# lightbulb128/troy

Hardware: AMD Instinct MI355X
Metric: ct x ct multiply+relinearize ops/sec, BFV N=2^15 L=14; achieved HBM GB/s vs peak (higher is better)
Workload: dtype u64; 1 GPU; bfv_n32768_l14; scheme=BFV, N=32768, K=15, L=14, batch_per_gpu=256, parallelism=batch-shard x1, streams_per_gpu=2, Bsk=15, limb_transforms_per_op=443

## Files before the change

### troy_amd/csrc/bfly.h

```cpp
#pragma once
#include "modarith.h"

namespace troyhip {

struct PrimeConst { u64 p, two_p, three_p, four_p, negp; };
__device__ __forceinline__ PrimeConst make_prime_const(u64 p) { return PrimeConst{p, 2 * p, 3 * p, 4 * p, 0 - p}; }

__device__ __forceinline__ u32 lo32(u64 x) { return (u32)x; }
__device__ __forceinline__ u32 hi32(u64 x) { return (u32)(x >> 32); }
__device__ __forceinline__ u64 mk64(u32 lo, u32 hi) { return ((u64)hi << 32) | lo; }

#ifdef TROYHIP_CPU_EMUL
__device__ __forceinline__ void csub4(u64 (&x)[4], u64 m) { for (int i = 0; i < 4; i++) x[i] = x[i] >= m ? x[i] - m : x[i]; }
__device__ __forceinline__ void sub4(u64 (&r)[4], const u64 (&a)[4], const u64 (&b)[4]) { for (int i = 0; i < 4; i++) r[i] = a[i] - b[i]; }
__device__ __forceinline__ u64 mulhi_approx1(u64 y, u64 wq) {
    const u64 y0 = lo32(y), y1 = hi32(y), q0 = lo32(wq), q1 = hi32(wq);
    const u128 s = (u128)(y1 * q0) + (u128)(y0 * q1);
    return y1 * q1 + (u64)(s >> 32);
}
__device__ __forceinline__ void mulhi_approx4(u64 (&q)[4], const u64 (&y)[4], const Shoup (&w)[4]) { for (int i = 0; i < 4; i++) q[i] = mulhi_approx1(y[i], w[i].quo); }
__device__ __forceinline__ u64 mul_acc(u64 acc, u64 y, u64 w, u64 q, u64 negp) { return acc + w * y + q * negp; }
__device__ __forceinline__ void mulhi_approx4_u(u64 (&q)[4], const u64 (&y)[4], const Shoup (&w)[4]) { mulhi_approx4(q, y, w); }
__device__ __forceinline__ u64 mul_acc_u(u64 acc, u64 y, u64 w, u64 q, u64 negp) { return mul_acc(acc, y, w, q, negp); }
__device__ __forceinline__ u64 mul_acc0(u64 y, u64 w, u64 q, u64 negp) { return mul_acc(0, y, w, q, negp); }
// ... 254 lines not shown
#pragma unroll
    for (int i = 0; i < 4; i++) {
        const u32 q = (u32)(((u64)hi32(x[i]) * mu) >> 32);
        x[i] += (u64)q * c.negp;
    }
}
__device__ __forceinline__ void lite_reduce1(u64 &x, u32 mu, const PrimeConst &c) {
    const u32 q = (u32)(((u64)hi32(x) * mu) >> 32);
    x += (u64)q * c.negp;
}
struct LeanFinal { unsigned sh; u32 mu; };
__device__ __forceinline__ LeanFinal make_lean_final(u64 p, u64 cr1) {
    const int b = 64 - __builtin_clzll(p);
    return LeanFinal{(unsigned)(b - 26), (u32)(cr1 >> (58 - b))};
}
__device__ __forceinline__ void lean_final4(u64 (&x)[4], const LeanFinal f, const PrimeConst &c) {
#pragma unroll
    for (int i = 0; i < 4; i++) {
        const u32 q = (u32)(((u64)(u32)(x[i] >> f.sh) * f.mu) >> 32);
        x[i] += (u64)q * c.negp;
    }
    csub4(x, c.p);
}
template <int NV> __device__ __forceinline__ void lean_final(u64 (&x)[NV], const LeanFinal f, const PrimeConst &c) {
#pragma unroll
    for (int h = 0; h < NV / 4; h++) {
        u64 v[4] = {x[4 * h], x[4 * h + 1], x[4 * h + 2], x[4 * h + 3]};
        lean_final4(v, f, c);
#pragma unroll
        for (int i = 0; i < 4; i++) x[4 * h + i] = v[i];
    }
}
__device__ __forceinline__ void reduce4_from_8p(u64 (&x)[4], const PrimeConst &c) { csub4(x, c.four_p); csub4(x, c.two_p); csub4(x, c.p); }
__device__ __forceinline__ void reduce4_from_4p(u64 (&x)[4], const PrimeConst &c) { csub4(x, c.two_p); csub4(x, c.p); }


struct Acc128 { u32 a0, a1, a2, a3; };
// ... 81 lines not shown
```

### troy_amd/csrc/evaluator.cpp

```cpp
#include "evaluator.h"
#include "hostcrypto.h"
#include "kernels.h"
#include <algorithm>
#include <cmath>
#include <cstdlib>
#include <cstring>

namespace troyhip {

static bool tensor_fused() {
    static const bool v = [] { const char *e = probe_env("TROYHIP_TENSOR"); return !(e && e[0] == 's'); }();
    return v;
}
static bool ks_fused() {
    static const bool v = [] { const char *e = probe_env("TROYHIP_KS"); return !(e && e[0] == 's'); }();
    return v;
}

static bool ks_moddown_fused() {
    static const bool v = [] { const char *e = probe_env("TROYHIP_MODDOWN"); return !(e && e[0] == 's'); }();
    return v;
}

static bool corr_fused() {
// ... 141 lines not shown
    u64 new_cf = a.cf;
    const bool same = (a.data == b.data && a.bstride == b.bstride && sa == sb);
    auto dense = [&](u64 bstride, u64 words) { return batch == 1 || bstride == words; };

    if (c.scheme == SCHEME_BFV) {
        if (a.ntt || b.ntt) throw Error(ST_INVALID_ARGUMENT, "encrypted1 or encrypted2 cannot be in NTT form");
        const Level &lv = c.level(L);
        const int nb = (int)lv.rns.Bsk.size();
        const u64 bw = (u64)nb * N;
        const int sp = sa + sb;
        u64 *xq = c.arena.take(batch * sp * pw), *xb = c.arena.take(batch * sp * bw);
        u64 *dq = c.arena.take(batch * ds * pw), *db = c.arena.take(batch * ds * bw);
        const LimbMap bmap = c.ids_map(lv.bsk_ids);
        const bool merged = dense(a.bstride, (u64)sa * pw) && dense(b.bstride, (u64)sb * pw) && sa == 2 && sb == 2 && ntt2_tensor_supported(c.logn) && tensor_fused() &&
                            L + nb <= 64 && take_merged(c, batch * sp * (u64)(L + nb));
        bool all_done = false;
        if (merged) {
            const u64 mw = (u64)(L + nb) * N;
            std::vector<uint8_t> ids;
            for (int l = 0; l < L; l++) ids.push_back((uint8_t)l);
            ids.insert(ids.end(), lv.bsk_ids.begin(), lv.bsk_ids.end());
            const LimbMap mmap = c.ids_map(ids);
            u64 *X = xq, *D = dq;
            if (xb != xq + batch * sp * pw || db != dq + batch * ds * pw) throw Error(ST_LOGIC_ERROR, "multiply: the merged scratch is not contiguous (arena alignment changed?)");
            u64 *X_b = same ? X : X + batch * sa * mw;
            if (same || batch * sp > 65535) {
                launch_behz_extend(a.data, pw, X + (u64)L * N, mw, c.d_desc, *lv.behz, N, batch * sa, s);
                if (!same) launch_behz_extend(b.data, pw, X_b + (u64)L * N, mw, c.d_desc, *lv.behz, N, batch * sb, s);
            } else launch_behz_extend(a.data, pw, X + (u64)L * N, mw, c.d_desc, *lv.behz, N, batch * sp, s, b.data, batch * sa);
            launch_ntt2_tensor(X, a.data, X_b, b.data, D, c.d_desc, mmap, batch, c.logn, s, (unsigned)L);
            const PrimeDesc *idesc = behz_floor_prescaled(*lv.behz) ? lv.behz->floor_desc : c.d_desc;
            launch_ntt(D, idesc, mmap, batch * ds * (u64)(L + nb), c.logn, true, s);
            u64 *res = dense(out.bstride, (u64)ds * pw) ? out.data : X;
            launch_behz_floor_sk(D, mw, D + (u64)L * N, mw, res, pw, c.d_desc, *lv.behz, N, batch * ds, s);
            if (res != out.data) launch_copy_strided(res, ds * pw, out.data, out.bstride, ds * pw, batch, s);
            all_done = true;
        } else if (dense(a.bstride, (u64)sa * pw) && dense(b.bstride, (u64)sb * pw)) {
            const bool fused = sa == 2 && sb == 2 && ntt2_tensor_supported(c.logn) && tensor_fused();
            const bool once = same && fused;
            u64 *xq_a = xq, *xq_b = once ? xq : xq + batch * sa * pw, *xb_a = xb, *xb_b = once ? xb : xb + batch * sa * bw;
            launch_behz_extend(a.data, pw, xb_a, bw, c.d_desc, *lv.behz, N, batch * sa, s);
            if (!once) launch_behz_extend(b.data, pw, xb_b, bw, c.d_desc, *lv.behz, N, batch * sb, s);
            if (fused) {
                launch_ntt2_tensor(xq_a, a.data, xq_b, b.data, dq, c.d_desc, qmap, batch, c.logn, s);
                launch_ntt2_tensor(xb_a, nullptr, xb_b, nullptr, db, c.d_desc, bmap, batch, c.logn, s);
            } else {
                launch_ntt_from(xq_a, a.data, c.d_desc, qmap, batch * sa * L, c.logn, s);
                launch_ntt_from(xq_b, b.data, c.d_desc, qmap, batch * sb * L, c.logn, s);
                launch_ntt(xb, c.d_desc, bmap, batch * sp * nb, c.logn, false, s);
                launch_tensor(sa, sb, xq_a, xq_b, dq, sa * pw, sb * pw, c.d_desc, qmap, c.logn, L, batch, s);
                launch_tensor(sa, sb, xb_a, xb_b, db, sa * bw, sb * bw, c.d_desc, bmap, c.logn, nb, batch, s);
            }
        } else {
            launch_copy_strided(a.data, a.bstride, xq, sp * pw, sa * pw, batch, s);
            launch_copy_strided(b.data, b.bstride, xq + sa * pw, sp * pw, sb * pw, batch, s);
            launch_behz_extend(xq, pw, xb, bw, c.d_desc, *lv.behz, N, batch * sp, s);
            launch_ntt(xq, c.d_desc, qmap, batch * sp * L, c.logn, false, s);
            launch_ntt(xb, c.d_desc, bmap, batch * sp * nb, c.logn, false, s);
            launch_tensor(sa, sb, xq, xq + sa * pw, dq, sp * pw, sp * pw, c.d_desc, qmap, c.logn, L, batch, s);
            launch_tensor(sa, sb, xb, xb + sa * bw, db, sp * bw, sp * bw, c.d_desc, bmap, c.logn, nb, batch, s);
        }
        if (!all_done) {
            const PrimeDesc *idesc = behz_floor_prescaled(*lv.behz) ? lv.behz->floor_desc : c.d_desc;
            launch_ntt(dq, idesc, qmap, batch * ds * L, c.logn, true, s);
            launch_ntt(db, idesc, bmap, batch * ds * nb, c.logn, true, s);
        }
        if (all_done) {
        } else if (dense(out.bstride, (u64)ds * pw)) {
            launch_behz_floor_sk(dq, pw, db, bw, out.data, pw, c.d_desc, *lv.behz, N, batch * ds, s);
        } else {
            u64 *res = xq;
            launch_behz_floor_sk(dq, pw, db, bw, res, pw, c.d_desc, *lv.behz, N, batch * ds, s);
            launch_copy_strided(res, ds * pw, out.data, out.bstride, ds * pw, batch, s);
        }
    } else if (c.scheme == SCHEME_CKKS) {
        if (!(a.ntt && b.ntt)) throw Error(ST_INVALID_ARGUMENT, "encrypted1 or encrypted2 must be in NTT form");
        new_scale = a.scale * b.scale;
        if (!scale_ok(new_scale, L)) throw Error(ST_INVALID_ARGUMENT, "scale out of bounds");
        if (out.data != a.data && out.data != b.data && dense(out.bstride, (u64)ds * pw)) {
            launch_tensor(sa, sb, a.data, b.data, out.data, a.bstride, b.bstride, c.d_desc, qmap, c.logn, L, batch, s);
// ... 673 lines not shown
```

### troy_amd/csrc/kernels.h

```cpp
#pragma once
#include "device_types.h"

namespace troyhip {

unsigned device_cus();
inline unsigned plan_per_workgroup(size_t units, unsigned cap, size_t groups) {
    const size_t want = 4 * (size_t)device_cus();
    unsigned r = cap ? cap : 1;
    while (r > 1 && ((units + r - 1) / r) * groups < want) r = (r + 1) / 2;
    return r;
}

void launch_ntt(u64 *data, const PrimeDesc *primes, const LimbMap &map, size_t rows, int logn, bool inverse, hipStream_t stream);
bool ntt2_tensor_supported(int logn);
bool ntt2_ks_mac_supported(int logn);
void launch_ntt2_tensor(u64 *xa, const u64 *src_a, u64 *xb, const u64 *src_b, u64 *out, const PrimeDesc *primes, const LimbMap &map, size_t batch, int logn,
                        hipStream_t stream, unsigned src_slots = 0);
void launch_ntt_from(u64 *data, const u64 *src, const PrimeDesc *primes, const LimbMap &map, size_t rows, int logn, hipStream_t stream);

struct KsBase { const u64 *ptr = nullptr; u64 bstride = 0; int polys = 1; };

bool ntt2_supported(int logn);
struct Ntt2ModDown { int kind; u64 *ct; u64 ct_bstride; unsigned dl; u64 qk, half; const u64 *share; KsBase base; };
enum class Ntt2Source {
    SAME_LAYOUT,
    KS_DIGITS
};
enum class Ntt2Passes { BOTH, FIRST, SECOND };
enum : unsigned { NTT_ALL_SLOTS = ~0u };
struct Ntt2Request {
    u64 *data;
    const PrimeDesc *primes;
    LimbMap map;
    size_t rows;
    int logn;
    bool inverse = false;
    struct {
        const u64 *ptr = nullptr;
        Ntt2Source kind = Ntt2Source::SAME_LAYOUT;
        u64 ostride = 0;
        u64 bound = 0;
    } src;
    unsigned slot_begin = 0, slot_count = NTT_ALL_SLOTS;
    Ntt2Passes passes = Ntt2Passes::BOTH;
    unsigned plan_begin = 0, plan_count = 0;
    const Ntt2ModDown *md = nullptr;
};
void launch_ntt2(const Ntt2Request &r, hipStream_t stream);
struct KsArgs;
void launch_ntt2_ks_mac(u64 *D, const u64 *src, u64 src_ostride, const LimbMap &map, size_t rows, const u64 *key, u64 *acc, const u64 *ckks_target, u64 t_bstride,
                        bool lazy, u64 src_bound, const KsArgs &a, hipStream_t stream);

enum class Ntt1Feature { PLAIN , MOD_DOWN , CORRECTION , STRIDED_INVERSE };
bool ntt1_supported(int logn, const LimbMap &map, size_t rows, Ntt1Feature feature = Ntt1Feature::PLAIN);
struct Ntt1ModDown { u64 *ct; u64 ct_bstride; u64 dl, qk, half; KsBase base; };
struct Ntt1Corr {
    const u64 *last, *in;
    u64 in_ostride;
    u64 *out;
    u64 out_gstride, out_ostride;
    unsigned group;
// ... 3 lines not shown
    u64 in_gstride = 0;
    KsBase base;
};
struct Ntt1Request {
    const PrimeDesc *primes;
    LimbMap map;
    size_t rows;
    int logn;
    u64 *data = nullptr;
    bool inverse = false;
    const u64 *src = nullptr;
    u64 src_ostride = 0;
    u64 slot_mask = ~0ull;
    const Ntt1ModDown *md = nullptr;
    const Ntt1Corr *cr = nullptr;
};
void launch_ntt1(const Ntt1Request &r, hipStream_t stream);

void launch_ew(int op, const u64 *a, const u64 *b, u64 *out, const PrimeDesc *primes, const LimbMap &map, int logn, u64 rows, hipStream_t s);
void launch_mul_scalar(u64 *x, const PrimeDesc *primes, const LimbMap &map, const u64 *scalars, int logn, u64 rows, hipStream_t s);
void launch_mul_plain(u64 *a, const u64 *plain, const PrimeDesc *primes, const LimbMap &map, int logn, u64 limbs, u64 rows, hipStream_t s,
                      u64 rows_per_item = 0, u64 plain_bstride = 0);

struct PlainArgs {
    const PrimeDesc *primes;
    LimbMap map;
    u64 delta[64];
    u64 t_p, t_cr0, t_cr1;
    u64 q_mod_t, thr;
    u64 cf;
// ... 211 lines not shown
```

### troy_amd/csrc/ntt.hip

```cpp
#include "kernels.h"

namespace troyhip {

struct NttArgs {
    u64 *data;
    const PrimeDesc *primes;
    LimbMap map;
    int logn;
    int logT;
    int s_first;
    int n_stages;
    int logC;
    int lps;
    int strided;
    int tiles_per_row_log;
    int final_pass;
};

#define NTT_THREADS 256

__device__ __forceinline__ u64 gidx(const NttArgs &a, unsigned tile, unsigned f) {
    unsigned base = a.strided ? (tile << a.logC) : (tile << a.logT);
    return ((u64)(f >> a.logC) << a.lps) + base + (f & ((1u << a.logC) - 1));
}
// ... 126 lines not shown
            }
            v.x = v.x >= p ? v.x - p : v.x;
            v.y = v.y >= p ? v.y - p : v.y;
        }
        *reinterpret_cast<ulonglong2 *>(x + gidx(a, tile, f)) = v;
    }
}

static void plan(int logn, int &k1, int &k2) {
    if (logn <= 11) { k1 = 0; k2 = logn; return; }
    k2 = 9;
    if (logn - k2 > 7) k2 = logn - 7;
    k1 = logn - k2;
}

static bool launch_production(u64 *data, const u64 *src, const PrimeDesc *primes, const LimbMap &map, size_t rows, int logn, bool inverse, hipStream_t stream) {
    if (ntt1_supported(logn, map, rows)) {
        Ntt1Request q{primes, map, rows, logn};
        q.data = data;
        q.src = src;
        q.inverse = inverse;
        launch_ntt1(q, stream);
        return true;
    }
    if (!ntt2_supported(logn) || rows % ((size_t)map.period * map.inner)) return false;
    Ntt2Request q{data, primes, map, rows, logn};
    q.src.ptr = src;
    q.inverse = inverse;
    launch_ntt2(q, stream);
    return true;
}
void launch_ntt_from(u64 *data, const u64 *src, const PrimeDesc *primes, const LimbMap &map, size_t rows, int logn, hipStream_t stream) {
    if (rows == 0 || launch_production(data, src, primes, map, rows, logn, false, stream)) return;
    HIP_CHECK(hipMemcpyAsync(data, src, (rows << logn) * sizeof(u64), hipMemcpyDeviceToDevice, stream));
    launch_ntt(data, primes, map, rows, logn, false, stream);
}
void launch_ntt(u64 *data, const PrimeDesc *primes, const LimbMap &map, size_t rows, int logn, bool inverse, hipStream_t stream) {
    if (rows == 0 || launch_production(data, nullptr, primes, map, rows, logn, inverse, stream)) return;
    int k1, k2;
    plan(logn, k1, k2);
    NttArgs a;
    a.data = data;
    a.primes = primes;
    a.map = map;
    a.logn = logn;
    a.logT = logn < 11 ? logn : 11;
    a.tiles_per_row_log = logn - a.logT;
    unsigned blocks = (unsigned)(rows << a.tiles_per_row_log);
    auto strided = [&](bool final_pass) {
        a.strided = 1; a.n_stages = k1; a.logC = a.logT - k1; a.lps = logn - k1; a.final_pass = final_pass;
        a.s_first = inverse ? k1 - 1 : 0;
    };
    auto contiguous = [&](bool final_pass) {
// ... 18 lines not shown
```

### troy_amd/csrc/ntt1.hip

```cpp
#include "kernels.h"
#include <atomic>
#include "bfly.h"
#include "fpmod.h"
#include <cstdio>
#include <cstdlib>
#include <cstring>
#include <type_traits>

namespace troyhip {

#define N1_THREADS 1024
#define N1_LOGN 15
#define N1_N (1u << N1_LOGN)

struct Ntt1Args {
    u64 *data;
    const u64 *src;
    u64 src_ostride;
    const PrimeDesc *primes;
    LimbMap map;
    unsigned m_total;
    unsigned rows_per_wg;
    unsigned chunks;
    unsigned nslots;
// ... 1033 lines not shown
        else return ntt1s_fwd_kernel<LOGN, LEAN>;
    }
}
void launch_ntt1(const Ntt1Request &r, hipStream_t stream) {
    const LimbMap &map = r.map;
    const int logn = r.logn;
    const bool inverse = r.inverse;
    const Ntt1ModDown *md = r.md;
    const Ntt1Corr *cr = r.cr;
    if (r.rows == 0) return;
    if (logn < 12 || logn > N1_LOGN) throw Error(ST_LOGIC_ERROR, "ntt1: unsupported size");
    if (logn != N1_LOGN && (cr || (r.src && inverse))) throw Error(ST_LOGIC_ERROR, "ntt1: the correction form and the strided source belong to N = 2^15");
    const size_t per_outer = (size_t)map.period * map.inner;
    if (r.rows % per_outer) throw Error(ST_INVALID_ARGUMENT, "ntt1: row count must be a multiple of the limb pattern");
    if (md && (!inverse || map.inner != 1 || md->dl >= map.period)) throw Error(ST_LOGIC_ERROR, "ntt1: the mod-down epilogue belongs to the inverse transform of [..][slot][N] accumulators");
    Ntt1Args a;
    std::memset(&a, 0, sizeof(a));
    a.data = r.data;
    a.src = r.src;
    a.src_ostride = r.src_ostride;
    if (r.src && inverse && !r.src_ostride) throw Error(ST_LOGIC_ERROR, "ntt1: the out-of-place inverse takes a strided source");
    a.primes = r.primes;
    a.map = map;
    a.m_total = (unsigned)(r.rows / per_outer * map.inner);
    if (cr) {
        if (inverse || map.inner != 1 || r.src) throw Error(ST_LOGIC_ERROR, "ntt1: the correction form belongs to the forward transform of [outer][slot][N] rows");
        a.cr_last = cr->last; a.cr_in = cr->in; a.cr_out = cr->out; a.cr_inv = cr->inv;
        a.cr_in_ostride = cr->in_ostride; a.cr_in_gstride = cr->in_gstride; a.cr_out_gstride = cr->out_gstride; a.cr_out_ostride = cr->out_ostride;
        a.cr_qx = cr->qx; a.cr_half = cr->half; a.cr_group = cr->group ? cr->group : 1; a.cr_accumulate = cr->accumulate ? 1 : 0;
        a.cr_base = cr->base.ptr; a.cr_base_gstride = cr->base.bstride; a.cr_base_polys = cr->base.polys;
// ... 88 lines not shown
```

### troy_amd/csrc/ntt2.hip

```cpp
#include "kernels.h"
#include "bfly.h"
#include "fpmod.h"
#include <cstdio>
#include <cstdlib>
#include <cstring>
#include <type_traits>

namespace troyhip {

#define N2_THREADS 256
#define N2_LOGT 11
#define N2_T 2048

struct Ntt2Args {
    u64 *data;
    const u64 *src;
    u64 src_ostride;
    const PrimeDesc *primes;
    LimbMap map;
    int logn;
    unsigned tiles_per_row_log;
    unsigned m_total;
    unsigned rows_per_wg;
    unsigned chunks;
    int src_reduce;
    u64 src_bound;
    int slot_fastest;
    int src_same_layout;
    const u64 *src2;
    unsigned src_slots, src_split;
    u64 *tensor_b;
    u64 *tensor_out;
    const u64 *mac_key;
    u64 *mac_acc;
    const u64 *mac_target;
    u64 mac_tstride;
    unsigned mac_K;
    int mac_lazy;
    uint8_t mac_key_limb[65];
    unsigned slot_begin = 0;
    u64 *md_ct = nullptr;
    u64 md_ct_bstride = 0, md_qk = 0, md_half = 0;
    const u64 *md_share = nullptr;
    const u64 *md_base = nullptr;
    u64 md_base_bstride = 0;
    int md_base_polys = 1;
    int skip_diag = 0;
// ... 208 lines not shown
    __device__ static __forceinline__ void stage_read(u64 (&x)[8], const u64 *wave_stage) {
        const unsigned lane = threadIdx.x & 63;
        if (INV) {
            const u64 *mine = wave_stage + 128 * (lane >> 4) + 2 * (lane & 15);
#pragma unroll
            for (int j = 0; j < 4; j++) {
                const ulonglong2 v = *reinterpret_cast<const ulonglong2 *>(mine + 32 * j);
                x[2 * j] = v.x;
                x[2 * j + 1] = v.y;
            }
        } else {
#pragma unroll
            for (int e = 0; e < 8; e++) x[e] = wave_stage[lane + 64 * e];
        }
    }
    __device__ static __forceinline__ void store_via_lds(const u64 (&x)[8], u64 *row, unsigned tile, u64 *wave_xchg) {
        const unsigned lane = threadIdx.x & 63, w = threadIdx.x >> 6;
        u64 *mine = wave_xchg + 128 * (lane >> 4) + 2 * (lane & 15);
#pragma unroll
        for (int j = 0; j < 4; j++) {
            ulonglong2 v;
            v.x = x[2 * j];
            v.y = x[2 * j + 1];
            *reinterpret_cast<ulonglong2 *>(mine + 32 * j) = v;
        }
        TROY_WAVE_SYNC();
        u64 *dst = row + ((size_t)tile << N2_LOGT) + 512 * w + 2 * unit_perm(lane);
#pragma unroll
        for (int c = 0; c < 4; c++) {
            const ulonglong2 v = *reinterpret_cast<const ulonglong2 *>(wave_xchg + 128 * c + 2 * lane);
            *reinterpret_cast<ulonglong2 *>(dst + 128 * c) = v;
        }
    }
    __device__ static __forceinline__ void tensor_epilogue(u64 (&x)[8], u64 (&tx)[3][8], unsigned mm, u64 *out, unsigned period, unsigned slot, unsigned tile, int logn,
                                                           const Mod &m, u64 *xchg, const bool lean, const FpPrime *fc = nullptr) {
        const PrimeConst pc = make_prime_const(m.p);
        if (fc) {
#pragma unroll
            for (int e = 0; e < 8; e++) x[e] = fp_canonical(fp_of_bits(x[e]), *fc, m.p);
        } else if (lean) {
#pragma unroll
            for (int h = 0; h < 2; h++) {
                u64 v[4] = {x[4 * h], x[4 * h + 1], x[4 * h + 2], x[4 * h + 3]};
                lite_reduce4(v, (u32)m.cr1, pc);
#pragma unroll
                for (int i = 0; i < 4; i++) x[4 * h + i] = v[i];
            }
        } else {
#pragma unroll
            for (int h = 0; h < 2; h++) {
                u64 v[4] = {x[4 * h], x[4 * h + 1], x[4 * h + 2], x[4 * h + 3]};
                reduce4_from_8p(v, pc);
#pragma unroll
                for (int i = 0; i < 4; i++) x[4 * h + i] = v[i];
            }
        }
        const unsigned vr = mm & 3;
        if (vr < 3) {
#pragma unroll
            for (int i = 0; i < 3; i++)
                if ((int)vr == i) {
#pragma unroll
                    for (int e = 0; e < 8; e++) tx[i][e] = x[e];
                }
            return;
        }
        const unsigned b = mm >> 2;
        const ProdMod pm = make_prod_mod(m);
        u64 d[3][8];
#pragma unroll
        for (int e = 0; e < 8; e++) {
            const u64 a0 = tx[0][e], a1 = tx[1][e], b0 = tx[2][e], b1 = x[e];
            d[0][e] = reduce_prod((u128)a0 * b0, pm);
            d[1][e] = reduce_prod((u128)a0 * b1 + (u128)a1 * b0, pm);
            d[2][e] = reduce_prod((u128)a1 * b1, pm);
        }
#pragma unroll
        for (int i = 0; i < 3; i++) {
            u64 *orow = out + ((((u64)b * 3 + i) * period + slot) << logn);
            if (xchg) {
                TROY_WAVE_SYNC();
                store_via_lds(d[i], orow, tile, xchg + 512 * (threadIdx.x >> 6));
                continue;
            }
            ulonglong2 *op = reinterpret_cast<ulonglong2 *>(orow + ((u64)tile << N2_LOGT) + 8 * threadIdx.x);
#pragma unroll
            for (int e = 0; e < 4; e++) {
                ulonglong2 v;
                v.x = d[i][2 * e];
                v.y = d[i][2 * e + 1];
                op[e] = v;
            }
        }
    }
    template <int REDUCE> __device__ static __forceinline__ void g_read(u64 (&x)[8], const u64 *row, unsigned tile, int logn, const Mod &m, const unsigned t = threadIdx.x) {
#pragma unroll
        for (int u = 0; u < G; u++) {
            const unsigned q = t + THREADS * u;
            if (LOGD == 0) {
#pragma unroll
                for (int e = 0; e < (1 << R); e += 2) {
                    const ulonglong2 v = *reinterpret_cast<const ulonglong2 *>(row + g_index<STRIDED, NS, LOGC>(tile, elem(q, e), logn));
                    x[(u << R) + e] = v.x;
                    x[(u << R) + e + 1] = v.y;
                }
// ... 180 lines not shown
        }
        const u64 r = ((u64)o * period + slot) * inner + k;
        row = a.data + (r << logn);
        in = (REDUCE || a.src) ? (a.src_same_layout ? a.src + (r << logn) : a.src + (u64)o * a.src_ostride + ((u64)k << logn)) : row;
        if constexpr (!REDUCE && STRIDED && !INV) {
            if (a.src_same_layout == 2)
                in = slot >= a.src_slots ? row : (o < a.src_split ? a.src + (((u64)o * a.src_slots + slot) << logn) : a.src2 + (((u64)(o - a.src_split) * a.src_slots + slot) << logn));
        }
    };
    constexpr bool DMA = WAVE_PRIVATE;
    static_assert(MAC != 3 || DMA, "the CKKS key-switch pass (MAC = 3) takes its rows from the LDS-DMA staging area");
    constexpr bool PF = STRIDED && !INV && NR == 2 && !REDUCE;
    u64 xn[PF ? 8 : 1];
    static_assert(!MAC || (!INV && !STRIDED && NS == 9), "the inner product is fused into the forward contiguous pass");
    u64 tx[MAC == 2 ? 3 : 1][8];
    Acc128 macc[2][2][4];
    double facc[2][FP ? 8 : 1];
    auto mac_row = [&](const u64 (&xr)[8], const ulonglong2 (&kw)[2][KS ? 4 : 1], unsigned row_no) {
        if constexpr (FP && KS) {
#pragma unroll
            for (int cpt = 0; cpt < 2; cpt++)
#pragma unroll
                for (int e = 0; e < 8; e++) {
                    const u64 kword = (e & 1) ? kw[cpt][e >> 1].y : kw[cpt][e >> 1].x;
                    facc[cpt][e] += fp_mulmod_pinv(fp_of_bits(xr[e]), fp_from_u64(kword), fc);
                }
            if (a.fp_acc_every && (row_no + 1) % a.fp_acc_every == 0) {
#pragma unroll
                for (int cpt = 0; cpt < 2; cpt++)
#pragma unroll
// ... 2 lines not shown
        } else if constexpr (KS) {
#pragma unroll
            for (int cpt = 0; cpt < 2; cpt++) {
#pragma unroll
                for (int g = 0; g < 2; g++) {
                    const ulonglong2 k01 = kw[cpt][2 * g], k23 = kw[cpt][2 * g + 1];
                    const u64 kk[4] = {k01.x, k01.y, k23.x, k23.y};
                    const u64 xx[4] = {xr[4 * g], xr[4 * g + 1], xr[4 * g + 2], xr[4 * g + 3]};
                    mac128x4(macc[cpt][g], xx, kk);
                }
            }
        }
        (void)row_no;
    };
    constexpr bool MAC_STORE_LINEAR = KS && WAVE_PRIVATE;
    u64 *const wave_stage = lds[1] + 512 * (threadIdx.x >> 6);
    constexpr bool KSU = MAC != 0 && !FP;
    const unsigned units = KSU ? (a.mac_units ? a.mac_units : 1u) : 1u;
    const unsigned groups = KSU && a.mac_groups ? a.mac_groups : a.chunks * units;
    const unsigned last_group = chunk * units + units < groups ? chunk * units + units : groups;
    const unsigned stage_end = KSU ? last_group * a.rows_per_wg : 0;
    for (unsigned un = 0; un < units; un++) {
        const unsigned uchunk = KSU ? chunk * units + un : chunk;
        if (KSU && uchunk >= groups) break;
        const unsigned m_begin = uchunk * a.rows_per_wg;
        const unsigned m_end = (m_begin + a.rows_per_wg < a.m_total) ? m_begin + a.rows_per_wg : a.m_total;
        if (KS) {
#pragma unroll
            for (int cpt = 0; cpt < 2; cpt++)
#pragma unroll
                for (int g = 0; g < 2; g++)
// ... 132 lines not shown
                        Rd0::template g_read<REDUCE>(xn, nin, tile, logn, m, n2_opaque(threadIdx.x));
                    }
                }
                fp_guard(x, 1);
                if constexpr (FP) Rd1::compute_fp(x, tw1, fc, pd.inv_n); else Rd1::compute(x, tw1, pd, lean);
                if constexpr (NR == 2) {
                    if constexpr (FINAL >= 3) Rd1::template md_write<FINAL>(x, a, mm, slot, tile, logn, m, pd, fcp);
                    else Rd1::template g_write<FINAL>(x, row, tile, logn, m, lean, nullptr, fcp);
                } else {
                    Rd1::lds_write(x, buf, (FRESH & 4) ? n2_opaque(threadIdx.x) : threadIdx.x);
                    round_sync();
                    Rd2::lds_read(x, buf, (FRESH & 8) ? n2_opaque(threadIdx.x) : threadIdx.x);
                    fp_guard(x, 2);
                    if constexpr (FP) Rd2::compute_fp(x, tw2, fc, pd.inv_n); else Rd2::compute(x, tw2, pd, lean);
                    if constexpr (NR == 3 && MAC == 2) {
                        Rd2::tensor_epilogue(x, tx, mm, a.tensor_out, period, slot, tile, logn, m, WAVE_PRIVATE ? buf : nullptr, lean, fcp);
                    } else if constexpr (NR == 3 && KS) {
                        if constexpr (FP) {
                        } else if (!a.mac_lazy && lean) {
#pragma unroll
                            for (int e = 0; e < 8; e++) x[e] = barrett64(x[e], m);
                        } else if (!a.mac_lazy) {
                            const PrimeConst pc = make_prime_const(pd.p);
#pragma unroll
                            for (int h = 0; h < 2; h++) {
                                u64 v[4] = {x[4 * h], x[4 * h + 1], x[4 * h + 2], x[4 * h + 3]};
                                reduce4_from_8p(v, pc);
#pragma unroll
                                for (int i = 0; i < 4; i++) x[4 * h + i] = v[i];
                            }
                        }
// ... 28 lines not shown
            if (!skip_row) parity ^= 1u;
        }
        if constexpr (KS) {
            const unsigned o = m_begin / inner;
            static_assert(!KS || MAC_STORE_LINEAR, "the sums leave through the wave's exchange area");
#pragma unroll
            for (int cpt = 0; cpt < 2; cpt++) {
                u64 lin[8];
                if constexpr (FP) {
#pragma unroll
                    for (int e = 0; e < 8; e++) lin[e] = fp_canonical(facc[cpt][e], fc, m.p);
                } else if (pd.p >> 33) {
                    const PrimeConst pc = make_prime_const(pd.p);
                    const LeanFinal lf = lean ? make_lean_final(pd.p, pd.cr1) : LeanFinal{0, 0};
                    const Shoup r64 = to_sgpr(pd.r64);
                    const Shoup w4[4] = {r64, r64, r64, r64};
#pragma unroll
                    for (int g = 0; g < 2; g++) {
                        u64 lo[4], hi[4], q[4];
#pragma unroll
                        for (int i = 0; i < 4; i++) {
                            const Acc128 &sum = macc[cpt][g][i];
                            lo[i] = mk64(sum.a0, sum.a1);
                            hi[i] = mk64(sum.a2, sum.a3);
                        }
                        lite_reduce4(lo, (u32)pd.cr1, pc);
                        mulhi_approx4_u(q, hi, w4);
#pragma unroll
                        for (int i = 0; i < 4; i++) lo[i] = mul_acc_u(lo[i], hi[i], r64.op, q[i], pc.negp);
                        if (lean) lean_final4(lo, lf, pc); else reduce4_from_8p(lo, pc);
#pragma unroll
                        for (int i = 0; i < 4; i++) lin[4 * g + i] = lo[i];
                    }
                } else {
#pragma unroll
                    for (int e = 0; e < 8; e++) {
                        const Acc128 &sum = macc[cpt][e >> 2][e & 3];
                        lin[e] = barrett128(mk64(sum.a0, sum.a1), mk64(sum.a2, sum.a3), m);
                    }
                }
                if constexpr (MAC_STORE_LINEAR) {
                    TROY_WAVE_SYNC();
                    Rd2::store_via_lds(lin, a.mac_acc + ((((u64)o * 2 + cpt) * period + slot) << logn), tile, lds[0] + 512 * (threadIdx.x >> 6));
                }
// ... 157 lines not shown
    const LimbMap &map = r.map;
    const Ntt2ModDown *md = r.md;
    const unsigned slot_begin = r.slot_begin, slot_count = r.slot_count == NTT_ALL_SLOTS ? map.period : r.slot_count;
    const bool inverse = r.inverse, run_first = r.passes != Ntt2Passes::SECOND, run_second = r.passes != Ntt2Passes::FIRST;
    if (r.plan_count && r.plan_begin + r.plan_count > map.period) throw Error(ST_INVALID_ARGUMENT, "ntt2: plan slot range");
    if (r.rows == 0 || slot_count == 0) return;
    if (slot_begin + slot_count > map.period) throw Error(ST_INVALID_ARGUMENT, "ntt2: slot range");
    const bool partial = slot_begin != 0 || slot_count != map.period;
    if ((partial || md || r.passes != Ntt2Passes::BOTH) && (!inverse || r.src.ptr)) throw Error(ST_LOGIC_ERROR, "ntt2: slot ranges, single passes and the mod-down epilogue belong to the in-place inverse transform");
    if (md && !run_second) throw Error(ST_LOGIC_ERROR, "ntt2: the mod-down epilogue rides on the second pass");
    if (md && map.inner != 1) throw Error(ST_LOGIC_ERROR, "ntt2: the mod-down epilogue takes one row per (item, prime)");
    if (!ntt2_supported(r.logn)) throw Error(ST_LOGIC_ERROR, "ntt2: unsupported size");
    const size_t per_outer = (size_t)map.period * map.inner;
    if (r.rows % per_outer) throw Error(ST_INVALID_ARGUMENT, "ntt2: row count must be a multiple of the limb pattern");
    if (r.src.ptr && inverse) throw Error(ST_LOGIC_ERROR, "ntt2: out-of-place input is only supported by the forward transform");
    int k1, k2;
    stage_split(r.logn, k1, k2);
    Ntt2Args a = common_args(r.data, r.primes, map, r.logn, r.rows / per_outer * map.inner);
    set_rows_per_wg(a, a.m_total < 8 ? a.m_total : (map.inner > 1 ? (map.inner <= 16 ? map.inner : 8) : 8), slot_count);
    a.slot_begin = slot_begin;
    a.md_base_polys = 1;
    if (md) {
        a.md_ct = md->ct; a.md_ct_bstride = md->ct_bstride; a.md_dl = md->dl; a.md_qk = md->qk; a.md_half = md->half;
        a.md_share = md->share;
        a.md_base = md->base.ptr; a.md_base_bstride = md->base.bstride; a.md_base_polys = md->base.polys;
        if (md->kind == 2 && !md->share) throw Error(ST_LOGIC_ERROR, "ntt2: the BGV mod-down needs the special limb's shares");
    }
    const bool digits = r.src.ptr && r.src.kind == Ntt2Source::KS_DIGITS;
    static const int md_order = [] { const char *e = probe_env("TROYHIP_NTT2_MD_ORDER"); return e ? std::atoi(e) : 1; }();
    ClassPlan cls[2];
// ... 67 lines not shown
        if (!fp) stats::counter(stats::KS_INT_GROUPS_PER_WG).fetch_add(second.mac_units, std::memory_order_relaxed);
        second.mac_key = key; second.mac_acc = acc; second.mac_target = ckks_target; second.mac_tstride = t_bstride; second.mac_K = (unsigned)ks.K;
        second.mac_lazy = lazy;
        std::memcpy(second.mac_key_limb, ks.key_limb, map.period);
        with_stages(logn - 9, 9, [&](auto ns1, auto) {
            launch_strided<0, decltype(ns1)::value>(first, true, stream, fp, -1, skip_diag);
            if (skip_diag) launch_one<0, 0, 9, 0, 1, 0, 3>(second, stream, fp);
            else launch_one<0, 0, 9, 0, 1, 0, 1>(second, stream, fp);
        });
    }
}

bool ntt2_tensor_supported(int logn) { return ntt2_supported(logn) && logn - 9 >= 3 && logn - 9 <= 7; }
bool ntt2_ks_mac_supported(int logn) { return ntt2_tensor_supported(logn); }
void launch_ntt2_tensor(u64 *xa, const u64 *src_a, u64 *xb, const u64 *src_b, u64 *out, const PrimeDesc *primes, const LimbMap &map, size_t batch, int logn,
                        hipStream_t stream, unsigned src_slots) {
    if (!batch) return;
    if (!ntt2_tensor_supported(logn) || map.inner != 1) throw Error(ST_LOGIC_ERROR, "ntt2 tensor: unsupported shape");
    const bool same = xa == xb;
    const bool joint = src_slots && !same && xb == xa + ((batch * 2 * map.period) << logn);
    if (src_slots && (!src_a || !src_b || src_slots > map.period)) throw Error(ST_LOGIC_ERROR, "ntt2 tensor: operands of the merged form");
    ClassPlan cls[2];
    const int ncls = plan_classes(map, 0, map.period, map.host_primes != nullptr, false, logn - 9, 9, 0, 0, 0, cls);
    for (int c = 0; c < ncls; c++) {
        const ClassPlan &k = cls[c];
        const bool fp = k.fp;
        stats::counter(fp ? stats::NTT2_FP_LAUNCHES : stats::NTT2_INT_LAUNCHES).fetch_add(1, std::memory_order_relaxed);
        with_stages(logn - 9, 9, [&](auto ns1, auto) {
            for (int part = 0; part < (same || joint ? 1 : 2); part++) {
                Ntt2Args a = common_args(part ? xb : xa, primes, map, logn, batch * (joint ? 4 : 2));
                const u64 *src = part ? src_b : src_a;
                set_class(a, k, k.mask1);
                set_rows_per_wg(a, a.m_total < 8 ? a.m_total : 8, k.nsel);
                if (src_slots) { a.src = src; a.src2 = src_b; a.src_same_layout = 2; a.src_slots = src_slots; a.src_split = joint ? (unsigned)(batch * 2) : ~0u; }
                else if (src) { a.src = src; a.src_same_layout = 1; }
                launch_strided<0, decltype(ns1)::value>(a, false, stream, fp);
            }
        });
        Ntt2Args a = common_args(xa, primes, map, logn, batch * 4);
        a.tensor_b = xb; a.tensor_out = out;
        set_class(a, k, k.mask2);
        a.rows_per_wg = 4;
        a.mac_groups = (unsigned)batch;
        a.mac_units = fp ? 1 : 4;
        while (a.mac_units > 1 && (size_t)((a.mac_groups + a.mac_units - 1) / a.mac_units) * ((size_t)k.nsel << a.tiles_per_row_log) < 12 * (size_t)device_cus()) a.mac_units >>= 1;
        a.chunks = (a.mac_groups + a.mac_units - 1) / a.mac_units;
        launch_one<0, 0, 9, 0, 1, 0, 2>(a, stream, fp);
    }
}

}
```

Measured before the change: 9879 ops/s.

## Use lazy Barrett fold in tensor epilogue and accept [0,2p) inverse-NTT inputs

In the fused forward-NTT plus tensor-product kernel, each 128-bit product is now reduced with a cheap fold plus lazy Barrett step, leaving values in [0,2p) instead of reducing them fully. Callers mark the following inverse NTT with a lazy entry bound, so the partly reduced values can flow straight into it. The epilogue also computes and stores one output polynomial at a time instead of holding all three, and the wave index is made uniform. The aim is to cut ALU work and register pressure in the epilogue. The cost is reliance on the inverse NTT tolerating inputs below 2p: the new entry-bound flag is only validated, not acted on in the kernels.

```diff
diff --git a/troy_amd/csrc/bfly.h b/troy_amd/csrc/bfly.h
--- a/troy_amd/csrc/bfly.h
+++ b/troy_amd/csrc/bfly.h
@@ -292,13 +292,28 @@
     const int b = 64 - __builtin_clzll(p);
     return LeanFinal{(unsigned)(b - 26), (u32)(cr1 >> (58 - b))};
 }
-__device__ __forceinline__ void lean_final4(u64 (&x)[4], const LeanFinal f, const PrimeConst &c) {
+__device__ __forceinline__ LeanFinal make_lazy_final(const Mod &m) {
+    const int b = 64 - __builtin_clzll(m.p);
+    return LeanFinal{(unsigned)(b - 26), b <= 58 ? (u32)(m.cr1 >> (58 - b)) : (u32)((m.cr1 << (b - 58)) | (m.cr0 >> (122 - b)))};
+}
+__device__ __forceinline__ void lean_lazy4(u64 (&x)[4], const LeanFinal f, const PrimeConst &c) {
 #pragma unroll
     for (int i = 0; i < 4; i++) {
         const u32 q = (u32)(((u64)(u32)(x[i] >> f.sh) * f.mu) >> 32);
         x[i] += (u64)q * c.negp;
     }
+}
+__device__ __forceinline__ void lean_final4(u64 (&x)[4], const LeanFinal f, const PrimeConst &c) {
+    lean_lazy4(x, f, c);
     csub4(x, c.p);
+}
+__device__ __forceinline__ void fold128x4(u64 (&lo)[4], const u64 (&hi)[4], const Shoup r64, u32 mu, const PrimeConst &c) {
+    const Shoup w4[4] = {r64, r64, r64, r64};
+    u64 q[4];
+    lite_reduce4(lo, mu, c);
+    mulhi_approx4_u(q, hi, w4);
+#pragma unroll
+    for (int i = 0; i < 4; i++) lo[i] = mul_acc_u(lo[i], hi[i], r64.op, q[i], c.negp);
 }
 template <int NV> __device__ __forceinline__ void lean_final(u64 (&x)[NV], const LeanFinal f, const PrimeConst &c) {
 #pragma unroll
diff --git a/troy_amd/csrc/evaluator.cpp b/troy_amd/csrc/evaluator.cpp
--- a/troy_amd/csrc/evaluator.cpp
+++ b/troy_amd/csrc/evaluator.cpp
@@ -179,7 +179,7 @@
         const LimbMap bmap = c.ids_map(lv.bsk_ids);
         const bool merged = dense(a.bstride, (u64)sa * pw) && dense(b.bstride, (u64)sb * pw) && sa == 2 && sb == 2 && ntt2_tensor_supported(c.logn) && tensor_fused() &&
                             L + nb <= 64 && take_merged(c, batch * sp * (u64)(L + nb));
-        bool all_done = false;
+        bool all_done = false, lazy_d = false;
         if (merged) {
             const u64 mw = (u64)(L + nb) * N;
             std::vector<uint8_t> ids;
@@ -193,9 +193,9 @@
                 launch_behz_extend(a.data, pw, X + (u64)L * N, mw, c.d_desc, *lv.behz, N, batch * sa, s);
                 if (!same) launch_behz_extend(b.data, pw, X_b + (u64)L * N, mw, c.d_desc, *lv.behz, N, batch * sb, s);
             } else launch_behz_extend(a.data, pw, X + (u64)L * N, mw, c.d_desc, *lv.behz, N, batch * sp, s, b.data, batch * sa);
-            launch_ntt2_tensor(X, a.data, X_b, b.data, D, c.d_desc, mmap, batch, c.logn, s, (unsigned)L);
+            launch_ntt2_tensor(X, a.data, X_b, b.data, D, c.d_desc, mmap, batch, c.logn, s, (unsigned)L, true);
             const PrimeDesc *idesc = behz_floor_prescaled(*lv.behz) ? lv.behz->floor_desc : c.d_desc;
-            launch_ntt(D, idesc, mmap, batch * ds * (u64)(L + nb), c.logn, true, s);
+            launch_ntt(D, idesc, mmap, batch * ds * (u64)(L + nb), c.logn, true, s, NTT_LAZY_ENTRY);
             u64 *res = dense(out.bstride, (u64)ds * pw) ? out.data : X;
             launch_behz_floor_sk(D, mw, D + (u64)L * N, mw, res, pw, c.d_desc, *lv.behz, N, batch * ds, s);
             if (res != out.data) launch_copy_strided(res, ds * pw, out.data, out.bstride, ds * pw, batch, s);
@@ -207,8 +207,9 @@
             launch_behz_extend(a.data, pw, xb_a, bw, c.d_desc, *lv.behz, N, batch * sa, s);
             if (!once) launch_behz_extend(b.data, pw, xb_b, bw, c.d_desc, *lv.behz, N, batch * sb, s);
             if (fused) {
-                launch_ntt2_tensor(xq_a, a.data, xq_b, b.data, dq, c.d_desc, qmap, batch, c.logn, s);
-                launch_ntt2_tensor(xb_a, nullptr, xb_b, nullptr, db, c.d_desc, bmap, batch, c.logn, s);
+                launch_ntt2_tensor(xq_a, a.data, xq_b, b.data, dq, c.d_desc, qmap, batch, c.logn, s, 0, true);
+                launch_ntt2_tensor(xb_a, nullptr, xb_b, nullptr, db, c.d_desc, bmap, batch, c.logn, s, 0, true);
+                lazy_d = true;
             } else {
                 launch_ntt_from(xq_a, a.data, c.d_desc, qmap, batch * sa * L, c.logn, s);
                 launch_ntt_from(xq_b, b.data, c.d_desc, qmap, batch * sb * L, c.logn, s);
@@ -227,8 +228,8 @@
         }
         if (!all_done) {
             const PrimeDesc *idesc = behz_floor_prescaled(*lv.behz) ? lv.behz->floor_desc : c.d_desc;
-            launch_ntt(dq, idesc, qmap, batch * ds * L, c.logn, true, s);
-            launch_ntt(db, idesc, bmap, batch * ds * nb, c.logn, true, s);
+            launch_ntt(dq, idesc, qmap, batch * ds * L, c.logn, true, s, lazy_d ? NTT_LAZY_ENTRY : 1u);
+            launch_ntt(db, idesc, bmap, batch * ds * nb, c.logn, true, s, lazy_d ? NTT_LAZY_ENTRY : 1u);
         }
         if (all_done) {
         } else if (dense(out.bstride, (u64)ds * pw)) {
diff --git a/troy_amd/csrc/kernels.h b/troy_amd/csrc/kernels.h
--- a/troy_amd/csrc/kernels.h
+++ b/troy_amd/csrc/kernels.h
@@ -11,11 +11,12 @@
     return r;
 }
 
-void launch_ntt(u64 *data, const PrimeDesc *primes, const LimbMap &map, size_t rows, int logn, bool inverse, hipStream_t stream);
+enum : unsigned { NTT_LAZY_ENTRY = 2 };
+void launch_ntt(u64 *data, const PrimeDesc *primes, const LimbMap &map, size_t rows, int logn, bool inverse, hipStream_t stream, unsigned entry_bound = 1);
 bool ntt2_tensor_supported(int logn);
 bool ntt2_ks_mac_supported(int logn);
 void launch_ntt2_tensor(u64 *xa, const u64 *src_a, u64 *xb, const u64 *src_b, u64 *out, const PrimeDesc *primes, const LimbMap &map, size_t batch, int logn,
-                        hipStream_t stream, unsigned src_slots = 0);
+                        hipStream_t stream, unsigned src_slots = 0, bool lazy_out = false);
 void launch_ntt_from(u64 *data, const u64 *src, const PrimeDesc *primes, const LimbMap &map, size_t rows, int logn, hipStream_t stream);
 
 struct KsBase { const u64 *ptr = nullptr; u64 bstride = 0; int polys = 1; };
@@ -45,6 +46,7 @@
     Ntt2Passes passes = Ntt2Passes::BOTH;
     unsigned plan_begin = 0, plan_count = 0;
     const Ntt2ModDown *md = nullptr;
+    unsigned entry_bound = 1;
 };
 void launch_ntt2(const Ntt2Request &r, hipStream_t stream);
 struct KsArgs;
@@ -78,6 +80,7 @@
     u64 slot_mask = ~0ull;
     const Ntt1ModDown *md = nullptr;
     const Ntt1Corr *cr = nullptr;
+    unsigned entry_bound = 1;
 };
 void launch_ntt1(const Ntt1Request &r, hipStream_t stream);
 
diff --git a/troy_amd/csrc/ntt.hip b/troy_amd/csrc/ntt.hip
--- a/troy_amd/csrc/ntt.hip
+++ b/troy_amd/csrc/ntt.hip
@@ -164,12 +164,13 @@
     k1 = logn - k2;
 }
 
-static bool launch_production(u64 *data, const u64 *src, const PrimeDesc *primes, const LimbMap &map, size_t rows, int logn, bool inverse, hipStream_t stream) {
+static bool launch_production(u64 *data, const u64 *src, const PrimeDesc *primes, const LimbMap &map, size_t rows, int logn, bool inverse, hipStream_t stream, unsigned entry_bound = 1) {
     if (ntt1_supported(logn, map, rows)) {
         Ntt1Request q{primes, map, rows, logn};
         q.data = data;
         q.src = src;
         q.inverse = inverse;
+        q.entry_bound = entry_bound;
         launch_ntt1(q, stream);
         return true;
     }
@@ -177,6 +178,7 @@
     Ntt2Request q{data, primes, map, rows, logn};
     q.src.ptr = src;
     q.inverse = inverse;
+    q.entry_bound = entry_bound;
     launch_ntt2(q, stream);
     return true;
 }
@@ -185,8 +187,9 @@
     HIP_CHECK(hipMemcpyAsync(data, src, (rows << logn) * sizeof(u64), hipMemcpyDeviceToDevice, stream));
     launch_ntt(data, primes, map, rows, logn, false, stream);
 }
-void launch_ntt(u64 *data, const PrimeDesc *primes, const LimbMap &map, size_t rows, int logn, bool inverse, hipStream_t stream) {
-    if (rows == 0 || launch_production(data, nullptr, primes, map, rows, logn, inverse, stream)) return;
+void launch_ntt(u64 *data, const PrimeDesc *primes, const LimbMap &map, size_t rows, int logn, bool inverse, hipStream_t stream, unsigned entry_bound) {
+    if (entry_bound != 1 && (!inverse || entry_bound == 0 || entry_bound > NTT_LAZY_ENTRY)) throw Error(ST_LOGIC_ERROR, "ntt: entry bound");
+    if (rows == 0 || launch_production(data, nullptr, primes, map, rows, logn, inverse, stream, entry_bound)) return;
     int k1, k2;
     plan(logn, k1, k2);
     NttArgs a;
diff --git a/troy_amd/csrc/ntt1.hip b/troy_amd/csrc/ntt1.hip
--- a/troy_amd/csrc/ntt1.hip
+++ b/troy_amd/csrc/ntt1.hip
@@ -1071,6 +1071,7 @@
     const size_t per_outer = (size_t)map.period * map.inner;
     if (r.rows % per_outer) throw Error(ST_INVALID_ARGUMENT, "ntt1: row count must be a multiple of the limb pattern");
     if (md && (!inverse || map.inner != 1 || md->dl >= map.period)) throw Error(ST_LOGIC_ERROR, "ntt1: the mod-down epilogue belongs to the inverse transform of [..][slot][N] accumulators");
+    if (r.entry_bound != 1 && (!inverse || cr || r.entry_bound == 0 || r.entry_bound > NTT_LAZY_ENTRY)) throw Error(ST_LOGIC_ERROR, "ntt1: entry bound");
     Ntt1Args a;
     std::memset(&a, 0, sizeof(a));
     a.data = r.data;
diff --git a/troy_amd/csrc/ntt2.hip b/troy_amd/csrc/ntt2.hip
--- a/troy_amd/csrc/ntt2.hip
+++ b/troy_amd/csrc/ntt2.hip
@@ -31,6 +31,7 @@
     unsigned src_slots, src_split;
     u64 *tensor_b;
     u64 *tensor_out;
+    int tensor_lazy;
     const u64 *mac_key;
     u64 *mac_acc;
     const u64 *mac_target;
@@ -269,8 +270,8 @@
             for (int e = 0; e < 8; e++) x[e] = wave_stage[lane + 64 * e];
         }
     }
-    __device__ static __forceinline__ void store_via_lds(const u64 (&x)[8], u64 *row, unsigned tile, u64 *wave_xchg) {
-        const unsigned lane = threadIdx.x & 63, w = threadIdx.x >> 6;
+    __device__ static __forceinline__ void store_via_lds(const u64 (&x)[8], u64 *row, unsigned tile, u64 *wave_xchg, const unsigned t = threadIdx.x) {
+        const unsigned lane = t & 63, w = t >> 6;
         u64 *mine = wave_xchg + 128 * (lane >> 4) + 2 * (lane & 15);
 #pragma unroll
         for (int j = 0; j < 4; j++) {
@@ -288,12 +289,13 @@
         }
     }
     __device__ static __forceinline__ void tensor_epilogue(u64 (&x)[8], u64 (&tx)[3][8], unsigned mm, u64 *out, unsigned period, unsigned slot, unsigned tile, int logn,
-                                                           const Mod &m, u64 *xchg, const bool lean, const FpPrime *fc = nullptr) {
+                                                           const Mod &m, u64 *xchg, const bool lean, const Shoup r64, const bool lazy, const FpPrime *fc = nullptr) {
         const PrimeConst pc = make_prime_const(m.p);
+        const bool fold = lazy && !fc && (m.p >> 33) != 0;
         if (fc) {
 #pragma unroll
             for (int e = 0; e < 8; e++) x[e] = fp_canonical(fp_of_bits(x[e]), *fc, m.p);
-        } else if (lean) {
+        } else if (fold || lean) {
 #pragma unroll
             for (int h = 0; h < 2; h++) {
                 u64 v[4] = {x[4 * h], x[4 * h + 1], x[4 * h + 2], x[4 * h + 3]};
@@ -321,29 +323,48 @@
             return;
         }
         const unsigned b = mm >> 2;
+        const LeanFinal lf = fold ? make_lazy_final(m) : LeanFinal{0, 0};
         const ProdMod pm = make_prod_mod(m);
-        u64 d[3][8];
-#pragma unroll
-        for (int e = 0; e < 8; e++) {
-            const u64 a0 = tx[0][e], a1 = tx[1][e], b0 = tx[2][e], b1 = x[e];
-            d[0][e] = reduce_prod((u128)a0 * b0, pm);
-            d[1][e] = reduce_prod((u128)a0 * b1 + (u128)a1 * b0, pm);
-            d[2][e] = reduce_prod((u128)a1 * b1, pm);
-        }
-#pragma unroll
-        for (int i = 0; i < 3; i++) {
-            u64 *orow = out + ((((u64)b * 3 + i) * period + slot) << logn);
-            if (xchg) {
+#pragma unroll
+        for (int j = 0; j < 3; j++) {
+            u64 *orow = out + ((((u64)b * 3 + j) * period + slot) << logn);
+            const unsigned t = n2_opaque(threadIdx.x);
+            u64 *const wx = xchg ? xchg + 512 * (t >> 6) : nullptr;
+            u64 d[8];
+            if (fold) {
+#pragma unroll
+                for (int h = 0; h < 2; h++) {
+                    u64 lo[4], hi[4];
+#pragma unroll
+                    for (int i = 0; i < 4; i++) {
+                        const u64 a0 = tx[0][4 * h + i], a1 = tx[1][4 * h + i], b0 = tx[2][4 * h + i], b1 = x[4 * h + i];
+                        const u128 pr = j == 0 ? (u128)a0 * b0 : j == 1 ? (u128)a0 * b1 + (u128)a1 * b0 : (u128)a1 * b1;
+                        lo[i] = (u64)pr;
+                        hi[i] = (u64)(pr >> 64);
+                    }
+                    fold128x4(lo, hi, r64, (u32)m.cr1, pc);
+                    lean_lazy4(lo, lf, pc);
+#pragma unroll
+                    for (int i = 0; i < 4; i++) d[4 * h + i] = lo[i];
+                }
+            } else {
+#pragma unroll
+                for (int e = 0; e < 8; e++) {
+                    const u64 a0 = tx[0][e], a1 = tx[1][e], b0 = tx[2][e], b1 = x[e];
+                    d[e] = reduce_prod(j == 0 ? (u128)a0 * b0 : j == 1 ? (u128)a0 * b1 + (u128)a1 * b0 : (u128)a1 * b1, pm);
+                }
+            }
+            if (wx) {
                 TROY_WAVE_SYNC();
-                store_via_lds(d[i], orow, tile, xchg + 512 * (threadIdx.x >> 6));
+                store_via_lds(d, orow, tile, wx, t);
                 continue;
             }
             ulonglong2 *op = reinterpret_cast<ulonglong2 *>(orow + ((u64)tile << N2_LOGT) + 8 * threadIdx.x);
 #pragma unroll
             for (int e = 0; e < 4; e++) {
                 ulonglong2 v;
-                v.x = d[i][2 * e];
-                v.y = d[i][2 * e + 1];
+                v.x = d[2 * e];
+                v.y = d[2 * e + 1];
                 op[e] = v;
             }
         }
@@ -554,6 +575,8 @@
     u64 xn[PF ? 8 : 1];
     static_assert(!MAC || (!INV && !STRIDED && NS == 9), "the inner product is fused into the forward contiguous pass");
     u64 tx[MAC == 2 ? 3 : 1][8];
+    const Shoup t_r64 = MAC == 2 ? to_sgpr(pd.r64) : Shoup{0, 0};
+    const bool t_lazy = MAC == 2 && __builtin_amdgcn_readfirstlane((int)(a.tensor_lazy && !((a.map.fp >> slot) & 1))) != 0;
     Acc128 macc[2][2][4];
     double facc[2][FP ? 8 : 1];
     auto mac_row = [&](const u64 (&xr)[8], const ulonglong2 (&kw)[2][KS ? 4 : 1], unsigned row_no) {
@@ -586,7 +609,7 @@
         (void)row_no;
     };
     constexpr bool MAC_STORE_LINEAR = KS && WAVE_PRIVATE;
-    u64 *const wave_stage = lds[1] + 512 * (threadIdx.x >> 6);
+    u64 *const wave_stage = lds[1] + 512 * (MAC == 2 ? (unsigned)__builtin_amdgcn_readfirstlane((int)(threadIdx.x >> 6)) : threadIdx.x >> 6);
     constexpr bool KSU = MAC != 0 && !FP;
     const unsigned units = KSU ? (a.mac_units ? a.mac_units : 1u) : 1u;
     const unsigned groups = KSU && a.mac_groups ? a.mac_groups : a.chunks * units;
@@ -749,7 +772,7 @@
                     fp_guard(x, 2);
                     if constexpr (FP) Rd2::compute_fp(x, tw2, fc, pd.inv_n); else Rd2::compute(x, tw2, pd, lean);
                     if constexpr (NR == 3 && MAC == 2) {
-                        Rd2::tensor_epilogue(x, tx, mm, a.tensor_out, period, slot, tile, logn, m, WAVE_PRIVATE ? buf : nullptr, lean, fcp);
+                        Rd2::tensor_epilogue(x, tx, mm, a.tensor_out, period, slot, tile, logn, m, WAVE_PRIVATE ? buf : nullptr, lean, t_r64, t_lazy, fcp);
                     } else if constexpr (NR == 3 && KS) {
                         if constexpr (FP) {
                         } else if (!a.mac_lazy && lean) {
@@ -808,20 +831,16 @@
                     const PrimeConst pc = make_prime_const(pd.p);
                     const LeanFinal lf = lean ? make_lean_final(pd.p, pd.cr1) : LeanFinal{0, 0};
                     const Shoup r64 = to_sgpr(pd.r64);
-                    const Shoup w4[4] = {r64, r64, r64, r64};
 #pragma unroll
                     for (int g = 0; g < 2; g++) {
-                        u64 lo[4], hi[4], q[4];
+                        u64 lo[4], hi[4];
 #pragma unroll
                         for (int i = 0; i < 4; i++) {
                             const Acc128 &sum = macc[cpt][g][i];
                             lo[i] = mk64(sum.a0, sum.a1);
                             hi[i] = mk64(sum.a2, sum.a3);
                         }
-                        lite_reduce4(lo, (u32)pd.cr1, pc);
-                        mulhi_approx4_u(q, hi, w4);
-#pragma unroll
-                        for (int i = 0; i < 4; i++) lo[i] = mul_acc_u(lo[i], hi[i], r64.op, q[i], pc.negp);
+                        fold128x4(lo, hi, r64, (u32)pd.cr1, pc);
                         if (lean) lean_final4(lo, lf, pc); else reduce4_from_8p(lo, pc);
 #pragma unroll
                         for (int i = 0; i < 4; i++) lin[4 * g + i] = lo[i];
@@ -1009,6 +1028,7 @@
     const size_t per_outer = (size_t)map.period * map.inner;
     if (r.rows % per_outer) throw Error(ST_INVALID_ARGUMENT, "ntt2: row count must be a multiple of the limb pattern");
     if (r.src.ptr && inverse) throw Error(ST_LOGIC_ERROR, "ntt2: out-of-place input is only supported by the forward transform");
+    if (r.entry_bound != 1 && (!inverse || r.entry_bound == 0 || r.entry_bound > NTT_LAZY_ENTRY)) throw Error(ST_LOGIC_ERROR, "ntt2: entry bound");
     int k1, k2;
     stage_split(r.logn, k1, k2);
     Ntt2Args a = common_args(r.data, r.primes, map, r.logn, r.rows / per_outer * map.inner);
@@ -1106,7 +1126,7 @@
 bool ntt2_tensor_supported(int logn) { return ntt2_supported(logn) && logn - 9 >= 3 && logn - 9 <= 7; }
 bool ntt2_ks_mac_supported(int logn) { return ntt2_tensor_supported(logn); }
 void launch_ntt2_tensor(u64 *xa, const u64 *src_a, u64 *xb, const u64 *src_b, u64 *out, const PrimeDesc *primes, const LimbMap &map, size_t batch, int logn,
-                        hipStream_t stream, unsigned src_slots) {
+                        hipStream_t stream, unsigned src_slots, bool lazy_out) {
     if (!batch) return;
     if (!ntt2_tensor_supported(logn) || map.inner != 1) throw Error(ST_LOGIC_ERROR, "ntt2 tensor: unsupported shape");
     const bool same = xa == xb;
@@ -1130,7 +1150,7 @@
             }
         });
         Ntt2Args a = common_args(xa, primes, map, logn, batch * 4);
-        a.tensor_b = xb; a.tensor_out = out;
+        a.tensor_b = xb; a.tensor_out = out; a.tensor_lazy = lazy_out;
         set_class(a, k, k.mask2);
         a.rows_per_wg = 4;
         a.mac_groups = (unsigned)batch;
```

Result: no change. 9911 ops/s, median of 6 (+0.3%).
